# zhoubin-me/agent0

Hardware: AMD Instinct MI355X
Metric: env-frames/sec (learner FPS: transitions collected and saved to replay per second with the learner running, pre-frameskip) (higher is better)
Workload: dtype f32

## Files before the change

### agent0_amd/csrc/conv1_wgrad.hip

```cpp
#include "a0_internal.h"

#include <cstdint>

typedef __bf16 a0w_bf16x8 __attribute__((ext_vector_type(8)));
typedef uint32_t a0w_u32x4 __attribute__((ext_vector_type(4)));
typedef float a0w_acc4 __attribute__((ext_vector_type(4)));

constexpr int A0W_THREADS = 512;
constexpr int A0W_XP_ROW = 24, A0W_XP_PLANE = 21 * 24;
constexpr int A0W_XP_ELEMS = 64 * A0W_XP_PLANE;
constexpr int A0W_T_PITCH = 488, A0W_T_TERM = 32 * A0W_T_PITCH;
constexpr int A0W_GROUPS = 60;
constexpr int A0W_STEPS = 15;

struct a0_c1w_args {
    const uint8_t* frames; const int* slot; long long sample_stride; int chan_off;
    const float* d1;
    float* slabs;
    int B;
};

A0_D uint32_t a0w_trunc(float f) { return __float_as_uint(f) >> 16; }
A0_D float a0w_up(uint32_t h) { return __uint_as_float(h << 16); }

__global__ __launch_bounds__(A0W_THREADS) void a0_conv1_wgrad_fused_kernel(a0_c1w_args P) {
    extern __shared__ __attribute__((aligned(16))) unsigned char smem[];
    uint16_t* Xp = (uint16_t*)smem;
    uint16_t* T = Xp + A0W_XP_ELEMS;
    const int tid = threadIdx.x, lane = tid & 63;
    const int wave = __builtin_amdgcn_readfirstlane(tid >> 6);
    const int q = lane >> 4, r16 = lane & 15;
    for (int i = tid; i < (A0W_XP_ELEMS + 3 * A0W_T_TERM) / 2; i += A0W_THREADS) ((uint32_t*)smem)[i] = 0u;
    int bbase[2], bshift[2];
#pragma unroll
    for (int t = 0; t < 2; ++t) {
        const int k = (2 * wave + t) * 16 + r16;
        const int c = k >> 6, kh = (k >> 3) & 7, kw = k & 7;
        const int plane = (c * 4 + (kh & 3)) * 4 + (kw & 3);
        bbase[t] = plane * A0W_XP_PLANE + (kh >> 2) * A0W_XP_ROW;
        bshift[t] = 2 * (kw >> 2);
    }
    a0w_acc4 acc[2][2];
#pragma unroll
    for (int i = 0; i < 2; ++i)
#pragma unroll
        for (int t = 0; t < 2; ++t) acc[i][t] = a0w_acc4{0.f, 0.f, 0.f, 0.f};
    float bsum = 0.f;
    __syncthreads();
    constexpr int NDW = 4 * 84 * 21, TR = (NDW + A0W_THREADS - 1) / A0W_THREADS;
    constexpr int GT = (A0W_GROUPS + A0W_THREADS / 32 - 1) / (A0W_THREADS / 32);
    uint32_t w[TR];
    float v[GT][8];
    auto load_raw = [&](int b) {
        const long long s = P.slot ? (long long)P.slot[b] : (long long)b;
        const uint32_t* src = (const uint32_t*)(P.frames + s * P.sample_stride + P.chan_off);
#pragma unroll
        for (int j = 0; j < TR; ++j) { const int i = tid + j * A0W_THREADS; w[j] = src[i < NDW ? i : NDW - 1]; }
        const float* g = P.d1 + (long long)b * 400 * 32 + (tid & 31);
#pragma unroll
        for (int t = 0; t < GT; ++t) {
            int G = (tid >> 5) + t * (A0W_THREADS / 32);
            G = G < A0W_GROUPS ? G : A0W_GROUPS - 1;
            const int oh = G / 3, ow0 = 8 * (G - 3 * oh);
#pragma unroll
            for (int j = 0; j < 8; ++j) { const int m = oh * 20 + ow0 + j; v[t][j] = g[(m < 400 ? m : 399) * 32]; }
        }
    };
    load_raw(blockIdx.x);
    for (int b = blockIdx.x; b < P.B; b += gridDim.x) {
#pragma unroll
        for (int j = 0; j < TR; ++j) {
            int i = tid + j * A0W_THREADS;
            i = i < NDW ? i : NDW - 1;
            const int c = i / (84 * 21), rem = i - c * (84 * 21), y = rem / 21, xc = rem - y * 21;
            uint16_t* d = Xp + ((c * 4 + (y & 3)) * 4) * A0W_XP_PLANE + (y >> 2) * A0W_XP_ROW + xc;
            d[0 * A0W_XP_PLANE] = (uint16_t)(__float_as_uint((float)(w[j] & 0xffu)) >> 16);
            d[1 * A0W_XP_PLANE] = (uint16_t)(__float_as_uint((float)((w[j] >> 8) & 0xffu)) >> 16);
            d[2 * A0W_XP_PLANE] = (uint16_t)(__float_as_uint((float)((w[j] >> 16) & 0xffu)) >> 16);
            d[3 * A0W_XP_PLANE] = (uint16_t)(__float_as_uint((float)(w[j] >> 24)) >> 16);
        }
        {
            const int n = tid & 31;
#pragma unroll
            for (int t = 0; t < GT; ++t) {
                const int G = (tid >> 5) + t * (A0W_THREADS / 32);
                if (G < A0W_GROUPS) {
                    const int oh = G / 3, ow0 = 8 * (G - 3 * oh);
                    uint32_t t0[4], t1[4], t2[4];
#pragma unroll
                    for (int j = 0; j < 8; j += 2) {
                        uint32_t h[2], m[2], l[2];
#pragma unroll
                        for (int e = 0; e < 2; ++e) {
                            const float x = (ow0 + j + e < 20) ? v[t][j + e] : 0.f;
                            bsum += x;
                            h[e] = a0w_trunc(x);
                            const float r1 = x - a0w_up(h[e]);
                            m[e] = a0w_trunc(r1);
                            l[e] = a0w_trunc(r1 - a0w_up(m[e]));
                        }
                        t0[j >> 1] = h[0] | (h[1] << 16); t1[j >> 1] = m[0] | (m[1] << 16); t2[j >> 1] = l[0] | (l[1] << 16);
                    }
                    uint16_t* d = T + n * A0W_T_PITCH + 8 * G;
                    *(uint4*)(d) = uint4{t0[0], t0[1], t0[2], t0[3]};
                    *(uint4*)(d + A0W_T_TERM) = uint4{t1[0], t1[1], t1[2], t1[3]};
                    *(uint4*)(d + 2 * A0W_T_TERM) = uint4{t2[0], t2[1], t2[2], t2[3]};
                }
            }
        }
        __syncthreads();
        if (b + (int)gridDim.x < P.B) load_raw(b + gridDim.x);
        {
            const uint16_t* ap = T + r16 * A0W_T_PITCH + 8 * q;
            const uint16_t* bp0 = Xp + bbase[0] + 8 * q;
            const uint16_t* bp1 = Xp + bbase[1] + 8 * q;
#pragma unroll 3
            for (int st = 0; st < A0W_STEPS; ++st) {
                a0w_u32x4 a[2][3], bf[2];
#pragma unroll
                for (int i = 0; i < 2; ++i)
#pragma unroll
                    for (int s3 = 0; s3 < 3; ++s3) {
                        const uint4 x = *(const uint4*)(ap + s3 * A0W_T_TERM + i * 16 * A0W_T_PITCH + 32 * st);
                        a[i][s3] = a0w_u32x4{x.x, x.y, x.z, x.w};
                    }
#pragma unroll
                for (int t = 0; t < 2; ++t) {
                    const uint16_t* bp = (t == 0 ? bp0 : bp1) + 32 * st;
                    const uint4 lo = *(const uint4*)bp;
                    const uint32_t hi = *(const uint32_t*)(bp + 8);
                    const int sh = bshift[t];
                    bf[t] = a0w_u32x4{__builtin_amdgcn_alignbyte(lo.y, lo.x, sh), __builtin_amdgcn_alignbyte(lo.z, lo.y, sh),
                                      __builtin_amdgcn_alignbyte(lo.w, lo.z, sh), __builtin_amdgcn_alignbyte(hi, lo.w, sh)};
                }
#pragma unroll
                for (int s3 = 0; s3 < 3; ++s3)
#pragma unroll
                    for (int i = 0; i < 2; ++i)
#pragma unroll
                        for (int t = 0; t < 2; ++t)
                            acc[i][t] = __builtin_amdgcn_mfma_f32_16x16x32_bf16(__builtin_bit_cast(a0w_bf16x8, a[i][s3]), __builtin_bit_cast(a0w_bf16x8, bf[t]), acc[i][t], 0, 0, 0);
            }
        }
        __syncthreads();
    }
    float* out = P.slabs + (long long)blockIdx.x * (32 * 256 + 32);
#pragma unroll
    for (int i = 0; i < 2; ++i)
#pragma unroll
        for (int t = 0; t < 2; ++t) {
            const int k = (2 * wave + t) * 16 + r16;
#pragma unroll
            for (int r = 0; r < 4; ++r) out[(i * 16 + 4 * q + r) * 256 + k] = acc[i][t][r] / 255.0f;
        }
    float* red = (float*)smem;
    red[tid] = bsum;
    __syncthreads();
    if (tid < 32) {
        float s = 0.f;
#pragma unroll
        for (int j = 0; j < A0W_THREADS / 32; ++j) s += red[j * 32 + tid];
        out[32 * 256 + tid] = s;
    }
}

int a0_conv1_wgrad_fused_launch(const a0_frames_arg* f, int C, int H, int W, int B, const float* d1, float* slabs, hipStream_t st) {
    if (C != 4 || H != 84 || W != 84 || B < 1 || (f->sample_stride & 3) || (f->chan_off & 3) || (((uintptr_t)f->frames) & 3)) return 0;
    a0_c1w_args P;
    P.frames = f->frames; P.slot = f->slot; P.sample_stride = f->sample_stride; P.chan_off = f->chan_off;
    P.d1 = d1; P.slabs = slabs; P.B = B;
    const int grid = B < 256 ? B : 256;
    const size_t lds = (size_t)(A0W_XP_ELEMS + 3 * A0W_T_TERM) * 2;
    static bool configured = false;
    if (!configured) {
        A0_HIP_THROW(hipFuncSetAttribute((const void*)a0_conv1_wgrad_fused_kernel, hipFuncAttributeMaxDynamicSharedMemorySize, (int)lds));
        configured = true;
    }
    hipLaunchKernelGGL(a0_conv1_wgrad_fused_kernel, dim3(grid), dim3(A0W_THREADS), lds, st, P);
    A0_HIP_THROW(hipGetLastError());
    return grid;
}
```

Before: 2.323 million.

## Split conv1 weight-grad sample into two halves and overlap staging with MFMA

Result: no change. 2.342 million, median of 6 (+0.8%).

```diff
diff --git a/agent0_amd/csrc/conv1_wgrad.hip b/agent0_amd/csrc/conv1_wgrad.hip
--- a/agent0_amd/csrc/conv1_wgrad.hip
+++ b/agent0_amd/csrc/conv1_wgrad.hip
@@ -1,17 +1,22 @@
 #include "a0_internal.h"
 
 #include <cstdint>
+#include <type_traits>
 
 typedef __bf16 a0w_bf16x8 __attribute__((ext_vector_type(8)));
 typedef uint32_t a0w_u32x4 __attribute__((ext_vector_type(4)));
 typedef float a0w_acc4 __attribute__((ext_vector_type(4)));
 
 constexpr int A0W_THREADS = 512;
-constexpr int A0W_XP_ROW = 24, A0W_XP_PLANE = 21 * 24;
+constexpr int A0W_XP_ROW = 24, A0W_XP_PLANE = 11 * A0W_XP_ROW;
 constexpr int A0W_XP_ELEMS = 64 * A0W_XP_PLANE;
-constexpr int A0W_T_PITCH = 488, A0W_T_TERM = 32 * A0W_T_PITCH;
-constexpr int A0W_GROUPS = 60;
-constexpr int A0W_STEPS = 15;
+constexpr int A0W_T_PITCH = 248, A0W_T_TERM = 32 * A0W_T_PITCH;
+constexpr int A0W_HALF = A0W_XP_ELEMS + 3 * A0W_T_TERM;
+constexpr int A0W_HGROUPS = 30;
+constexpr int A0W_STEPS = 15, A0W_STEP_B = 7;
+constexpr int A0W_HDW = 4 * 44 * 21;
+constexpr int A0W_TR = (A0W_HDW + A0W_THREADS - 1) / A0W_THREADS;
+constexpr int A0W_UNITS = 2 * A0W_TR;
 
 struct a0_c1w_args {
     const uint8_t* frames; const int* slot; long long sample_stride; int chan_off;
@@ -20,17 +25,23 @@
     int B;
 };
 
+struct a0w_frag { uint4 a[2][3]; uint4 lo[2]; uint32_t hi[2]; };
+
 A0_D uint32_t a0w_trunc(float f) { return __float_as_uint(f) >> 16; }
 A0_D float a0w_up(uint32_t h) { return __uint_as_float(h << 16); }
 
 __global__ __launch_bounds__(A0W_THREADS) void a0_conv1_wgrad_fused_kernel(a0_c1w_args P) {
     extern __shared__ __attribute__((aligned(16))) unsigned char smem[];
-    uint16_t* Xp = (uint16_t*)smem;
-    uint16_t* T = Xp + A0W_XP_ELEMS;
+    uint16_t* const buf0 = (uint16_t*)smem;
+    uint16_t* const buf1 = buf0 + A0W_HALF;
     const int tid = threadIdx.x, lane = tid & 63;
     const int wave = __builtin_amdgcn_readfirstlane(tid >> 6);
     const int q = lane >> 4, r16 = lane & 15;
-    for (int i = tid; i < (A0W_XP_ELEMS + 3 * A0W_T_TERM) / 2; i += A0W_THREADS) ((uint32_t*)smem)[i] = 0u;
+    for (int r = tid; r < 2 * 64 * 11; r += A0W_THREADS) {
+        const int h = r >= 64 * 11 ? 1 : 0;
+        uint16_t* d = buf0 + h * A0W_HALF + (r - h * 64 * 11) * A0W_XP_ROW + 21;
+        d[0] = 0; d[1] = 0; d[2] = 0;
+    }
     int bbase[2], bshift[2];
 #pragma unroll
     for (int t = 0; t < 2; ++t) {
@@ -40,108 +51,162 @@
         bbase[t] = plane * A0W_XP_PLANE + (kh >> 2) * A0W_XP_ROW;
         bshift[t] = 2 * (kw >> 2);
     }
+    int xoff[A0W_TR], goff[A0W_TR];
+    {
+        int c = 0, y = tid / 21, xc = tid - 21 * y;
+#pragma unroll
+        for (int j = 0; j < A0W_TR; ++j) {
+            const bool in = tid + j * A0W_THREADS < A0W_HDW;
+            const int cc = in ? c : 3, yy = in ? y : 43, xx = in ? xc : 20;
+            xoff[j] = ((cc * 4 + (yy & 3)) * 4) * A0W_XP_PLANE + (yy >> 2) * A0W_XP_ROW + xx;
+            goff[j] = cc * (84 * 21) + yy * 21 + xx;
+            xc += 8; y += 24;
+            if (xc >= 21) { xc -= 21; y += 1; }
+            if (y >= 44) { y -= 44; c += 1; }
+        }
+    }
+    const int n = tid & 31, g16 = tid >> 5;
+    int m0[2][2], nval[2][2], tdst[2][2];
+#pragma unroll
+    for (int h = 0; h < 2; ++h)
+#pragma unroll
+        for (int t = 0; t < 2; ++t) {
+            const int G = h == 0 ? g16 + 16 * t : g16 + 16 * ((g16 >= 14 ? 1 : 2) + t);
+            const bool ok = h == 0 ? G < A0W_HGROUPS : G < 2 * A0W_HGROUPS;
+            const int Gc = ok ? G : 2 * A0W_HGROUPS - 1;
+            const int oh = Gc / 3, g3 = Gc - 3 * oh;
+            m0[h][t] = Gc == 2 * A0W_HGROUPS - 1 ? 392 : oh * 20 + 8 * g3;
+            nval[h][t] = ok ? (g3 == 2 ? 4 : 8) : 0;
+            tdst[h][t] = n * A0W_T_PITCH + (ok ? 8 * (G - h * A0W_HGROUPS) : 8 * A0W_HGROUPS);
+        }
     a0w_acc4 acc[2][2];
 #pragma unroll
     for (int i = 0; i < 2; ++i)
 #pragma unroll
         for (int t = 0; t < 2; ++t) acc[i][t] = a0w_acc4{0.f, 0.f, 0.f, 0.f};
     float bsum = 0.f;
+    uint32_t w[A0W_TR];
+    float v[2][8];
+    struct a0w_src { const uint32_t* px; const float* g; };
+    auto source = [&](int b, int h) {
+        const long long s = P.slot ? (long long)P.slot[b] : (long long)b;
+        return a0w_src{(const uint32_t*)(P.frames + s * P.sample_stride + P.chan_off) + h * 40 * 21, P.d1 + (long long)b * 400 * 32 + n};
+    };
+    auto load_px = [&](const a0w_src& S, int j) { return S.px[goff[j]]; };
+    auto load_d1 = [&](const a0w_src& S, int h, int t, int j) { return (S.g + m0[h][t] * 32)[j * 32]; };
+    const bool last_group = g16 == 11;
+    uint32_t t0[4], t1[4], t2[4];
+    auto unit = [&](auto H, int u, uint16_t* hb, const int (&nv)[2], const a0w_src& N) {
+        constexpr int h = decltype(H)::value;
+        if ((u & 1) == 0) {
+            const int j = u >> 1;
+            const uint32_t x = w[j];
+            w[j] = load_px(N, j);
+            uint16_t* d = hb + xoff[j];
+            d[0 * A0W_XP_PLANE] = (uint16_t)(__float_as_uint((float)(x & 0xffu)) >> 16);
+            d[1 * A0W_XP_PLANE] = (uint16_t)(__float_as_uint((float)((x >> 8) & 0xffu)) >> 16);
+            d[2 * A0W_XP_PLANE] = (uint16_t)(__float_as_uint((float)((x >> 16) & 0xffu)) >> 16);
+            d[3 * A0W_XP_PLANE] = (uint16_t)(__float_as_uint((float)(x >> 24)) >> 16);
+        } else {
+            const int t = u >> 3, p = (u >> 1) & 3;
+            uint32_t hh[2], mm[2], ll[2];
+#pragma unroll
+            for (int e = 0; e < 2; ++e) {
+                float x = v[t][2 * p + e];
+                if (h == 1 && t == 1 && p < 2) x = last_group ? v[t][2 * p + e + 4] : x;
+                x = (2 * p + e < nv[t]) ? x : 0.f;
+                v[t][2 * p + e] = load_d1(N, 1 - h, t, 2 * p + e);
+                bsum += x;
+                hh[e] = a0w_trunc(x);
+                const float r1 = x - a0w_up(hh[e]);
+                mm[e] = a0w_trunc(r1);
+                ll[e] = a0w_trunc(r1 - a0w_up(mm[e]));
+            }
+            t0[p] = hh[0] | (hh[1] << 16); t1[p] = mm[0] | (mm[1] << 16); t2[p] = ll[0] | (ll[1] << 16);
+            if (p == 3) {
+                uint16_t* d = hb + A0W_XP_ELEMS + tdst[h][t];
+                *(uint4*)(d) = uint4{t0[0], t0[1], t0[2], t0[3]};
+                *(uint4*)(d + A0W_T_TERM) = uint4{t1[0], t1[1], t1[2], t1[3]};
+                *(uint4*)(d + 2 * A0W_T_TERM) = uint4{t2[0], t2[1], t2[2], t2[3]};
+            }
+        }
+    };
+    a0w_frag f;
+    auto read_a = [&](const uint16_t* hb, int off, int s3) {
+        const uint16_t* ap = hb + A0W_XP_ELEMS + r16 * A0W_T_PITCH + off + s3 * A0W_T_TERM;
+#pragma unroll
+        for (int i = 0; i < 2; ++i) f.a[i][s3] = *(const uint4*)(ap + i * 16 * A0W_T_PITCH);
+    };
+    auto read_b = [&](const uint16_t* hb, int off) {
+#pragma unroll
+        for (int t = 0; t < 2; ++t) {
+            const uint16_t* bp = hb + bbase[t] + off;
+            f.lo[t] = *(const uint4*)bp;
+            f.hi[t] = *(const uint32_t*)(bp + 8);
+        }
+    };
+    auto read_frag = [&](const uint16_t* hb, int off) {
+        read_b(hb, off);
+#pragma unroll
+        for (int s3 = 0; s3 < 3; ++s3) read_a(hb, off, s3);
+    };
+    auto phase = [&](auto H, const int (&nv)[2], const a0w_src& N) {
+        constexpr int h = decltype(H)::value;
+        constexpr int ST0 = h ? 0 : A0W_STEP_B, ST1 = h ? A0W_STEP_B : A0W_STEPS, NM = (ST1 - ST0) * 12;
+        uint16_t* const dst = h ? buf1 : buf0;
+#pragma unroll
+        for (int st = ST0; st < ST1; ++st) {
+            const bool next = st + 1 < ST1 || h;
+            const uint16_t* nb = (st + 1 < ST1 && !h) ? buf1 : buf0;
+            const int noff = st + 1 < ST1 ? 8 * (4 * (st + 1) + q) - (h ? 0 : 8 * A0W_HGROUPS) : 8 * (4 * A0W_STEP_B + (q & 1));
+            a0w_u32x4 bf[2];
+#pragma unroll
+            for (int t = 0; t < 2; ++t) {
+                const uint4 lo = f.lo[t];
+                const uint32_t hi = f.hi[t];
+                const int sh = bshift[t];
+                bf[t] = a0w_u32x4{__builtin_amdgcn_alignbyte(lo.y, lo.x, sh), __builtin_amdgcn_alignbyte(lo.z, lo.y, sh),
+                                  __builtin_amdgcn_alignbyte(lo.w, lo.z, sh), __builtin_amdgcn_alignbyte(hi, lo.w, sh)};
+            }
+            __builtin_amdgcn_sched_barrier(0);
+            if (next) read_b(nb, noff);
+            __builtin_amdgcn_sched_barrier(0);
+#pragma unroll
+            for (int m = 0; m < 12; ++m) {
+                const int s3 = m >> 2, i = (m >> 1) & 1, t = m & 1;
+                const uint4 x = f.a[i][s3];
+                acc[i][t] = __builtin_amdgcn_mfma_f32_16x16x32_bf16(__builtin_bit_cast(a0w_bf16x8, a0w_u32x4{x.x, x.y, x.z, x.w}), __builtin_bit_cast(a0w_bf16x8, bf[t]), acc[i][t], 0, 0, 0);
+                if ((m & 3) == 3 && next) read_a(nb, noff, s3);
+                const int mm = (st - ST0) * 12 + m;
+#pragma unroll
+                for (int u = mm * A0W_UNITS / NM; u < (mm + 1) * A0W_UNITS / NM; ++u) unit(H, u, dst, nv, N);
+                __builtin_amdgcn_sched_barrier(0);
+            }
+        }
+    };
+    const std::integral_constant<int, 0> H0;
+    const std::integral_constant<int, 1> H1;
+    {
+        const a0w_src S = source(blockIdx.x, 0), N = source(blockIdx.x, 1);
+#pragma unroll
+        for (int j = 0; j < A0W_TR; ++j) w[j] = load_px(S, j);
+#pragma unroll
+        for (int t = 0; t < 2; ++t)
+#pragma unroll
+            for (int j = 0; j < 8; ++j) v[t][j] = load_d1(S, 0, t, j);
+#pragma unroll
+        for (int u = 0; u < A0W_UNITS; ++u) unit(H0, u, buf0, nval[0], N);
+    }
     __syncthreads();
-    constexpr int NDW = 4 * 84 * 21, TR = (NDW + A0W_THREADS - 1) / A0W_THREADS;
-    constexpr int GT = (A0W_GROUPS + A0W_THREADS / 32 - 1) / (A0W_THREADS / 32);
-    uint32_t w[TR];
-    float v[GT][8];
-    auto load_raw = [&](int b) {
-        const long long s = P.slot ? (long long)P.slot[b] : (long long)b;
-        const uint32_t* src = (const uint32_t*)(P.frames + s * P.sample_stride + P.chan_off);
-#pragma unroll
-        for (int j = 0; j < TR; ++j) { const int i = tid + j * A0W_THREADS; w[j] = src[i < NDW ? i : NDW - 1]; }
-        const float* g = P.d1 + (long long)b * 400 * 32 + (tid & 31);
-#pragma unroll
-        for (int t = 0; t < GT; ++t) {
-            int G = (tid >> 5) + t * (A0W_THREADS / 32);
-            G = G < A0W_GROUPS ? G : A0W_GROUPS - 1;
-            const int oh = G / 3, ow0 = 8 * (G - 3 * oh);
-#pragma unroll
-            for (int j = 0; j < 8; ++j) { const int m = oh * 20 + ow0 + j; v[t][j] = g[(m < 400 ? m : 399) * 32]; }
-        }
-    };
-    load_raw(blockIdx.x);
     for (int b = blockIdx.x; b < P.B; b += gridDim.x) {
-#pragma unroll
-        for (int j = 0; j < TR; ++j) {
-            int i = tid + j * A0W_THREADS;
-            i = i < NDW ? i : NDW - 1;
-            const int c = i / (84 * 21), rem = i - c * (84 * 21), y = rem / 21, xc = rem - y * 21;
-            uint16_t* d = Xp + ((c * 4 + (y & 3)) * 4) * A0W_XP_PLANE + (y >> 2) * A0W_XP_ROW + xc;
-            d[0 * A0W_XP_PLANE] = (uint16_t)(__float_as_uint((float)(w[j] & 0xffu)) >> 16);
-            d[1 * A0W_XP_PLANE] = (uint16_t)(__float_as_uint((float)((w[j] >> 8) & 0xffu)) >> 16);
-            d[2 * A0W_XP_PLANE] = (uint16_t)(__float_as_uint((float)((w[j] >> 16) & 0xffu)) >> 16);
-            d[3 * A0W_XP_PLANE] = (uint16_t)(__float_as_uint((float)(w[j] >> 24)) >> 16);
-        }
-        {
-            const int n = tid & 31;
-#pragma unroll
-            for (int t = 0; t < GT; ++t) {
-                const int G = (tid >> 5) + t * (A0W_THREADS / 32);
-                if (G < A0W_GROUPS) {
-                    const int oh = G / 3, ow0 = 8 * (G - 3 * oh);
-                    uint32_t t0[4], t1[4], t2[4];
-#pragma unroll
-                    for (int j = 0; j < 8; j += 2) {
-                        uint32_t h[2], m[2], l[2];
-#pragma unroll
-                        for (int e = 0; e < 2; ++e) {
-                            const float x = (ow0 + j + e < 20) ? v[t][j + e] : 0.f;
-                            bsum += x;
-                            h[e] = a0w_trunc(x);
-                            const float r1 = x - a0w_up(h[e]);
-                            m[e] = a0w_trunc(r1);
-                            l[e] = a0w_trunc(r1 - a0w_up(m[e]));
-                        }
-                        t0[j >> 1] = h[0] | (h[1] << 16); t1[j >> 1] = m[0] | (m[1] << 16); t2[j >> 1] = l[0] | (l[1] << 16);
-                    }
-                    uint16_t* d = T + n * A0W_T_PITCH + 8 * G;
-                    *(uint4*)(d) = uint4{t0[0], t0[1], t0[2], t0[3]};
-                    *(uint4*)(d + A0W_T_TERM) = uint4{t1[0], t1[1], t1[2], t1[3]};
-                    *(uint4*)(d + 2 * A0W_T_TERM) = uint4{t2[0], t2[1], t2[2], t2[3]};
-                }
-            }
-        }
+        const bool more = b + (int)gridDim.x < P.B;
+        const int bn = more ? b + (int)gridDim.x : b;
+        read_frag(buf0, 8 * q);
+        phase(H1, nval[1], source(bn, 0));
         __syncthreads();
-        if (b + (int)gridDim.x < P.B) load_raw(b + gridDim.x);
-        {
-            const uint16_t* ap = T + r16 * A0W_T_PITCH + 8 * q;
-            const uint16_t* bp0 = Xp + bbase[0] + 8 * q;
-            const uint16_t* bp1 = Xp + bbase[1] + 8 * q;
-#pragma unroll 3
-            for (int st = 0; st < A0W_STEPS; ++st) {
-                a0w_u32x4 a[2][3], bf[2];
-#pragma unroll
-                for (int i = 0; i < 2; ++i)
-#pragma unroll
-                    for (int s3 = 0; s3 < 3; ++s3) {
-                        const uint4 x = *(const uint4*)(ap + s3 * A0W_T_TERM + i * 16 * A0W_T_PITCH + 32 * st);
-                        a[i][s3] = a0w_u32x4{x.x, x.y, x.z, x.w};
-                    }
-#pragma unroll
-                for (int t = 0; t < 2; ++t) {
-                    const uint16_t* bp = (t == 0 ? bp0 : bp1) + 32 * st;
-                    const uint4 lo = *(const uint4*)bp;
-                    const uint32_t hi = *(const uint32_t*)(bp + 8);
-                    const int sh = bshift[t];
-                    bf[t] = a0w_u32x4{__builtin_amdgcn_alignbyte(lo.y, lo.x, sh), __builtin_amdgcn_alignbyte(lo.z, lo.y, sh),
-                                      __builtin_amdgcn_alignbyte(lo.w, lo.z, sh), __builtin_amdgcn_alignbyte(hi, lo.w, sh)};
-                }
-#pragma unroll
-                for (int s3 = 0; s3 < 3; ++s3)
-#pragma unroll
-                    for (int i = 0; i < 2; ++i)
-#pragma unroll
-                        for (int t = 0; t < 2; ++t)
-                            acc[i][t] = __builtin_amdgcn_mfma_f32_16x16x32_bf16(__builtin_bit_cast(a0w_bf16x8, a[i][s3]), __builtin_bit_cast(a0w_bf16x8, bf[t]), acc[i][t], 0, 0, 0);
-            }
-        }
+        if (q >= 2) read_frag(buf1, 8 * (q - 2));
+        const int nv0[2] = {more ? nval[0][0] : 0, more ? nval[0][1] : 0};
+        phase(H0, nv0, source(bn, 1));
         __syncthreads();
     }
     float* out = P.slabs + (long long)blockIdx.x * (32 * 256 + 32);
@@ -170,7 +235,7 @@
     P.frames = f->frames; P.slot = f->slot; P.sample_stride = f->sample_stride; P.chan_off = f->chan_off;
     P.d1 = d1; P.slabs = slabs; P.B = B;
     const int grid = B < 256 ? B : 256;
-    const size_t lds = (size_t)(A0W_XP_ELEMS + 3 * A0W_T_TERM) * 2;
+    const size_t lds = (size_t)2 * A0W_HALF * 2;
     static bool configured = false;
     if (!configured) {
         A0_HIP_THROW(hipFuncSetAttribute((const void*)a0_conv1_wgrad_fused_kernel, hipFuncAttributeMaxDynamicSharedMemorySize, (int)lds));
```
